# google-research/rigl

Measured on AMD Instinct MI355X. Metric: images/sec/node, ResNet-50 80% ERK RigL step, higher is better.
Workload: dtype bf16

## Files before the change

include/rigl_hip.h:

```cpp
#ifndef RIGL_HIP_H_
#define RIGL_HIP_H_

#include <stddef.h>
#include <stdint.h>

#ifdef __cplusplus
extern "C" {
#endif

#define RIGL_ABI_VERSION 2

typedef void* rigl_stream_t;
typedef uint16_t rigl_bf16;

enum {
  RIGL_OK = 0,
  RIGL_EINVAL = -1,
  RIGL_ELAUNCH = -2,
  RIGL_EWORKSPACE = -3,
  RIGL_EUNSUPPORTED = -4
};

int rigl_version(void);
uint32_t rigl_crc32c(const void* data, size_t n, uint32_t crc);
// ... 383 lines not shown
                           void* workspace, size_t workspace_bytes, rigl_stream_t stream);
int rigl_bn_relu_maxpool_fwd(const RiglConvDesc* d, const rigl_bf16* x,
                             const float* scale, const float* shift, rigl_bf16* y,
                             uint8_t* argmax, rigl_stream_t stream);
size_t rigl_bn_relu_maxpool_bwd_workspace_bytes(const RiglConvDesc* d);
int rigl_bn_relu_maxpool_bwd(const RiglConvDesc* d, const rigl_bf16* x,
                             const rigl_bf16* dy, const uint8_t* argmax,
                             const float* gamma, const float* save_mean,
                             const float* save_invstd, const float* save_scale,
                             const float* save_shift, rigl_bf16* dx, float* dgamma,
                             float* dbeta, void* workspace, size_t workspace_bytes,
                             rigl_stream_t stream);

int rigl_global_avgpool_fwd(int32_t n, int32_t pixels, int32_t c, const rigl_bf16* x,
                            rigl_bf16* y, rigl_stream_t stream);
int rigl_global_avgpool_bwd(int32_t n, int32_t pixels, int32_t c, const rigl_bf16* dy,
                            rigl_bf16* dx, rigl_stream_t stream);
int rigl_global_avgpool_bwd_relu(int32_t n, int32_t pixels, int32_t c, const rigl_bf16* dy,
                                 const rigl_bf16* x, rigl_bf16* dx, rigl_stream_t stream);
int rigl_softmax_xent(int32_t rows, int32_t classes, const rigl_bf16* logits,
                      const int64_t* labels, float label_smoothing, float grad_scale,
                      float* row_loss, rigl_bf16* dlogits , rigl_stream_t stream);

int32_t rigl_conv2d_fwd_takes_relu_epilogue(const RiglConvDesc* d);
int32_t rigl_conv2d_bwd_takes_relu_epilogue(const RiglConvDesc* d);
int rigl_masked_conv2d_fwd_relu(const RiglConvDesc* d, const rigl_bf16* x,
                                const rigl_bf16* w_ohwi, rigl_bf16* y, void* workspace,
                                size_t workspace_bytes, rigl_stream_t stream);
int rigl_masked_conv2d_bwd_relu(const RiglConvDesc* d, const rigl_bf16* x,
                                const rigl_bf16* dy, const rigl_bf16* w_hwio, float* dw,
                                rigl_bf16* dx, void* workspace, size_t workspace_bytes,
                                rigl_stream_t stream);
int rigl_relu_fwd(int64_t n, const rigl_bf16* x, rigl_bf16* y, rigl_stream_t stream);
int rigl_relu_bwd(int64_t n, const rigl_bf16* dy, const rigl_bf16* x, rigl_bf16* dx,
                  rigl_stream_t stream);

typedef struct RiglBnInferItem {
  const float* gamma;
  const float* beta;
  const float* moving_mean;
  const float* moving_variance;
  float* scale_shift;
  int32_t c;
  float eps;
} RiglBnInferItem;
int rigl_bn_infer_params_batched(const RiglBnInferItem* items, int32_t n_items,
// ... 48 lines not shown
```

rigl_amd/_lib.py:

```python
import ctypes as C
import os

_HERE = os.path.dirname(os.path.abspath(__file__))
ABI_VERSION = 2
LIB_PATH = os.environ.get('RIGL_HIP_LIB') or os.path.join(_HERE, 'lib', 'librigl_hip.so')

RIGL_OK = 0
RIGL_EINVAL = -1
RIGL_ELAUNCH = -2
RIGL_EWORKSPACE = -3
RIGL_EUNSUPPORTED = -4
COUNTS_PER_LAYER = 8
MAGPRUNE_COUNTS_PER_LAYER = 4
PROF_KINDS = ('conv_fwd', 'conv_dgrad', 'conv_wgrad', 'prune_regrow',
              'sgd_momentum', 'pack_weights', 'conv_bwd', 'depthwise', 'masked_adam', 'magnitude_prune')

GROW_ZEROS, GROW_GRAD_SCALE, GROW_GRAD_SIGN, GROW_EXPLICIT = 0, 1, 2, 3
MOMRESET_ZEROS, MOMRESET_GRAD = 0, 1


class RiglError(RuntimeError):

  def __init__(self, code, msg):
    super().__init__('librigl_hip: error %d: %s' % (code, msg))
# ... 144 lines not shown
    'rigl_bn_bwd': (C.c_int, [_I64, _I32, _P, _P, _P, _P, _P, _P, _P, _P, _P, _I32, _P, _P, _P, _P, _P, _SZ, _P]),
    'rigl_bn_bwd_stats': (C.c_int, [_I64, _I32, _P, _P, _P, _P, _P, _P, _P, _P, _P, _I32, _P, _P, _P, _P, _P, _I32, _P, _SZ, _P]),
    'rigl_bn_bwd_reduce': (C.c_int, [_I64, _I32, _P, _P, _P, _P, _P, _P, _I32, _P, _P, _P, _P, _SZ, _P]),
    'rigl_crc32c': (C.c_uint32, [_P, _SZ, C.c_uint32]),
    'rigl_stateless_random': (C.c_int, [_P, _I64, _I32, _I32, _I32, _F, _F, _P]),
    'rigl_stateless_random_batched': (C.c_int, [C.POINTER(RandomItem), _I32, _P]),
    'rigl_dropout_fwd': (C.c_int, [_P, _P, _P, _I64, _I32, _F, _I32, _P, _P]),
    'rigl_dropout_bwd': (C.c_int, [_P, _P, _P, _I64, _I32, _F, _P]),
    'rigl_dropout_advance': (C.c_int, [_P, _P]),
    'rigl_cifar_batch': (C.c_int, [_P, _P, _I64, _I32, _I32, _I32, _I32, _I32, _P, _P, _I32, _P, _P, _P]),
    'rigl_cifar_advance': (C.c_int, [_P, _P]),
    'rigl_maxpool_fwd': (C.c_int, [C.POINTER(ConvDesc), _P, _P, _P, _P]),
    'rigl_maxpool_bwd': (C.c_int, [C.POINTER(ConvDesc), _P, _P, _P, _P]),
    'rigl_bn_fwd_statistics': (C.c_int, [_I64, _I32, _P, _P, _P, _P, _P, _F, _F, _P, _P, _P, _P, _P, _I32, _P, _SZ, _P]),
    'rigl_bn_add_bn_fwd': (C.c_int, [_I64, _I32, _P, _P, _P, _P, _P, _P, _P, _P, _F, _F, _I32, _P, _P, _P, _P, _P, _P, _I32, _P, _P, _SZ, _P]),
    'rigl_bn_add_bn_bwd_workspace_bytes': (_SZ, [_I64, _I32]),
    'rigl_bn_add_bn_bwd': (C.c_int, [_I64, _I32, _P, _P, _P, _P, _P, _P, _P, _P, _P, _P, _P, _P, _P, _P, _P, _P, _P, _SZ, _P]),
    'rigl_bn_relu_maxpool_fwd': (C.c_int, [C.POINTER(ConvDesc), _P, _P, _P, _P, _P, _P]),
    'rigl_bn_relu_maxpool_bwd_workspace_bytes': (_SZ, [C.POINTER(ConvDesc)]),
    'rigl_bn_relu_maxpool_bwd': (C.c_int, [C.POINTER(ConvDesc), _P, _P, _P, _P, _P, _P, _P, _P, _P, _P, _P, _P, _SZ, _P]),
    'rigl_global_avgpool_fwd': (C.c_int, [_I32, _I32, _I32, _P, _P, _P]),
    'rigl_global_avgpool_bwd': (C.c_int, [_I32, _I32, _I32, _P, _P, _P]),
    'rigl_softmax_xent': (C.c_int, [_I32, _I32, _P, _P, _F, _F, _P, _P, _P]),
    'rigl_global_avgpool_bwd_relu': (C.c_int, [_I32, _I32, _I32, _P, _P, _P, _P]),
    'rigl_conv2d_fwd_takes_relu_epilogue': (C.c_int32, [C.POINTER(ConvDesc)]),
    'rigl_conv2d_bwd_takes_relu_epilogue': (C.c_int32, [C.POINTER(ConvDesc)]),
    'rigl_masked_conv2d_fwd_relu': (C.c_int, [C.POINTER(ConvDesc), _P, _P, _P, _P, _SZ, _P]),
    'rigl_masked_conv2d_bwd_relu': (C.c_int, [C.POINTER(ConvDesc), _P, _P, _P, _P, _P, _P, _SZ, _P]),
    'rigl_relu_fwd': (C.c_int, [_I64, _P, _P, _P]),
    'rigl_relu_bwd': (C.c_int, [_I64, _P, _P, _P, _P]),
    'rigl_bn_infer_params_batched': (C.c_int, [C.POINTER(BnInferItem), _I32, _P]),
    'rigl_bn_apply': (C.c_int, [_I64, _I32, _P, _P, _P, _I32, _P, _P]),
    'rigl_bn_apply_pair': (C.c_int, [_I64, _I32, _P, _P, _P, _P, _I32, _P, _P]),
    'rigl_bn_relu_maxpool_infer': (C.c_int, [C.POINTER(ConvDesc), _P, _P, _P, _P]),
    'rigl_conv2d_fwd_takes_bn_epilogue': (C.c_int32, [C.POINTER(ConvDesc), _I32, _I32]),
    'rigl_masked_conv2d_fwd_bn_infer': (C.c_int, [C.POINTER(ConvDesc), _P, _P, _P, _P, _P, _I32, _P, _P]),
    'rigl_eval_metrics': (C.c_int, [_I32, _I32, _P, _P, _F, _I32, _P, _P, _P, _P]),
    'rigl_prof_enable': (C.c_int, [_I32]),
    'rigl_prof_collect': (C.c_int, [C.POINTER(C.c_double), C.POINTER(_I64)]),
    'rigl_prof_collect_kinds': (C.c_int, [C.POINTER(C.c_double), C.POINTER(_I64), _I32]),
    'rigl_prof_collect_launches': (C.c_int, [C.POINTER(ProfLaunch), _I64, C.POINTER(_I64)]),
    'rigl_probe_mfma_bf16': (C.c_int, [_I32, _I32, _P, _P]),
    'rigl_tune_set': (C.c_int, [C.c_char_p, _I32]),
    'rigl_tune_get': (_I32, [C.c_char_p, _I32]),
    'rigl_tune_generation': (C.c_uint64, []),
    'rigl_tune_generation_addr': (C.c_void_p, []),
# ... 34 lines not shown
```

rigl_amd/csrc/head.hip:

```cpp
#include "common.hpp"

namespace rigl {
namespace khead {

constexpr int THREADS = 256;

__device__ __forceinline__ float bf_lo(uint32_t v) { return __uint_as_float(v << 16); }
__device__ __forceinline__ float bf_hi(uint32_t v) { return __uint_as_float(v & 0xFFFF0000u); }
__device__ __forceinline__ uint32_t f2bf(float f) {
  uint32_t u = __float_as_uint(f);
  if ((u & 0x7FFFFFFFu) > 0x7F800000u) return (u >> 16) | 0x40u;
  u += 0x7FFFu + ((u >> 16) & 1u);
  return u >> 16;
}
__device__ __forceinline__ float bf16_at(const uint16_t* p, int64_t i) { return __uint_as_float((uint32_t)p[i] << 16); }

__global__ __launch_bounds__(THREADS) void k_avgpool_fwd(int n, int p, int c2, const uint32_t* __restrict__ x,
                                                          uint32_t* __restrict__ y) {
  const int i = blockIdx.x * THREADS + threadIdx.x;
  if (i >= n * c2) return;
  const int img = i / c2, ch = i % c2;
  const uint32_t* src = x + (int64_t)img * p * c2 + ch;
  float a = 0.f, b = 0.f;
  for (int q = 0; q < p; ++q) {
// ... 4 lines not shown
  y[i] = f2bf(a / inv) | (f2bf(b / inv) << 16);
}

__global__ __launch_bounds__(THREADS) void k_avgpool_fwd8(int n, int p, int c8, const uint4* __restrict__ x, uint4* __restrict__ y) {
  const int i = blockIdx.x * THREADS + threadIdx.x;
  if (i >= n * c8) return;
  const int img = i / c8, ch = i % c8;
  const uint4* src = x + (int64_t)img * p * c8 + ch;
  float a[8];
#pragma unroll
  for (int j = 0; j < 8; ++j) a[j] = 0.f;
#pragma unroll 7
  for (int q = 0; q < p; ++q) {
    const uint4 v = src[(int64_t)q * c8];
    a[0] += bf_lo(v.x); a[1] += bf_hi(v.x); a[2] += bf_lo(v.y); a[3] += bf_hi(v.y);
    a[4] += bf_lo(v.z); a[5] += bf_hi(v.z); a[6] += bf_lo(v.w); a[7] += bf_hi(v.w);
  }
  const float inv = (float)p;
  uint4 o;
  o.x = f2bf(a[0] / inv) | (f2bf(a[1] / inv) << 16); o.y = f2bf(a[2] / inv) | (f2bf(a[3] / inv) << 16);
  o.z = f2bf(a[4] / inv) | (f2bf(a[5] / inv) << 16); o.w = f2bf(a[6] / inv) | (f2bf(a[7] / inv) << 16);
  y[i] = o;
}
__global__ __launch_bounds__(THREADS) void k_avgpool_bwd8(int n, int p, int c8, const uint4* __restrict__ dy, uint4* __restrict__ dx) {
  const int64_t total = (int64_t)n * p * c8;
  const float inv = (float)p;
  for (int64_t i = (int64_t)blockIdx.x * THREADS + threadIdx.x; i < total; i += (int64_t)gridDim.x * THREADS) {
    const int ch = (int)(i % c8);
    const int img = (int)(i / ((int64_t)p * c8));
    const uint4 v = dy[(int64_t)img * c8 + ch];
    uint4 o;
    o.x = f2bf(bf_lo(v.x) / inv) | (f2bf(bf_hi(v.x) / inv) << 16); o.y = f2bf(bf_lo(v.y) / inv) | (f2bf(bf_hi(v.y) / inv) << 16);
    o.z = f2bf(bf_lo(v.z) / inv) | (f2bf(bf_hi(v.z) / inv) << 16); o.w = f2bf(bf_lo(v.w) / inv) | (f2bf(bf_hi(v.w) / inv) << 16);
    dx[i] = o;
  }
}

__global__ __launch_bounds__(THREADS) void k_avgpool_bwd8_relu(int n, int p, int c8, const uint4* __restrict__ dy,
                                                               const uint4* __restrict__ x, uint4* __restrict__ dx) {
  const int64_t total = (int64_t)n * p * c8;
  const float inv = (float)p;
  for (int64_t i0 = (int64_t)blockIdx.x * THREADS; i0 < total; i0 += (int64_t)gridDim.x * THREADS) {
    const int64_t i = i0 + threadIdx.x, c = i < total ? i : total - 1;
    const int ch = (int)(c % c8);
    const int img = (int)(c / ((int64_t)p * c8));
    const uint4 v = dy[(int64_t)img * c8 + ch], xv = x[c];
    uint4 o;
    o.x = f2bf(bf_lo(v.x) / inv) | (f2bf(bf_hi(v.x) / inv) << 16); o.y = f2bf(bf_lo(v.y) / inv) | (f2bf(bf_hi(v.y) / inv) << 16);
    o.z = f2bf(bf_lo(v.z) / inv) | (f2bf(bf_hi(v.z) / inv) << 16); o.w = f2bf(bf_lo(v.w) / inv) | (f2bf(bf_hi(v.w) / inv) << 16);
    if (i < total) dx[i] = gate_bf16x8(o, xv);
  }
}

__global__ __launch_bounds__(THREADS) void k_avgpool_bwd(int n, int p, int c2, const uint32_t* __restrict__ dy,
                                                          uint32_t* __restrict__ dx) {
  const int64_t total = (int64_t)n * p * c2;
  for (int64_t i = (int64_t)blockIdx.x * THREADS + threadIdx.x; i < total; i += (int64_t)gridDim.x * THREADS) {
// ... 111 lines not shown
  if ((threadIdx.x & 63) == 0) {
    const int w = threadIdx.x >> 6;
    shv[w] = bv; shi[w] = bi; shc[w] = greater | (nonfinite << 30);
  }
  __syncthreads();
  if (threadIdx.x == 0) {
    int cnt = shc[0] & 0x3FFFFFFF, nf = shc[0] >> 30;
    for (int w = 1; w < THREADS / 64; ++w) {
      if (am_better(shv[w], shi[w], bv, bi)) { bv = shv[w]; bi = shi[w]; }
      cnt += shc[w] & 0x3FFFFFFF; nf |= shc[w] >> 30;
    }
    const bool top1 = inr && bi == (int)lab;
    const bool topkh = inr && isfinite(zlab) && !nf && cnt < topk;
    row_loss[row] = xent_loss(lse, sz, inr ? zlab - m : 0.f, inr, k, 1.f - eps, eps / (float)k);
    row_flags[row] = (top1 ? 1 : 0) | (topkh ? 2 : 0);
    if (counts) {
      atomicAdd(counts, 1ull);
      if (top1) atomicAdd(counts + 1, 1ull);
      if (topkh) atomicAdd(counts + 2, 1ull);
    }
  }
}

}
}

extern "C" {

int rigl_global_avgpool_fwd(int32_t n, int32_t pixels, int32_t c, const rigl_bf16* x, rigl_bf16* y, rigl_stream_t stream) {
  using namespace rigl;
  using namespace rigl::khead;
  if (n <= 0 || pixels <= 0 || c <= 0 || (c & 1)) return fail(RIGL_EINVAL, "rigl_global_avgpool_fwd: need n, pixels > 0 and an even channel count");
  if (!x || !y) return fail(RIGL_EINVAL, "rigl_global_avgpool_fwd: NULL tensor");
  const int c2 = c / 2;
  if ((c & 7) == 0 && ((uintptr_t)x & 15) == 0 && ((uintptr_t)y & 15) == 0) {
    const int c8 = c / 8;
    hipLaunchKernelGGL(k_avgpool_fwd8, dim3((unsigned)((n * c8 + THREADS - 1) / THREADS)), dim3(THREADS), 0, as_stream(stream),
                       n, pixels, c8, reinterpret_cast<const uint4*>(x), reinterpret_cast<uint4*>(y));
    RIGL_CHECK_LAUNCH("rigl_global_avgpool_fwd");
    return RIGL_OK;
  }
  hipLaunchKernelGGL(k_avgpool_fwd, dim3((unsigned)((n * c2 + THREADS - 1) / THREADS)), dim3(THREADS), 0, as_stream(stream),
                     n, pixels, c2, reinterpret_cast<const uint32_t*>(x), reinterpret_cast<uint32_t*>(y));
  RIGL_CHECK_LAUNCH("rigl_global_avgpool_fwd");
  return RIGL_OK;
}

int rigl_global_avgpool_bwd(int32_t n, int32_t pixels, int32_t c, const rigl_bf16* dy, rigl_bf16* dx, rigl_stream_t stream) {
  using namespace rigl;
  using namespace rigl::khead;
  if (n <= 0 || pixels <= 0 || c <= 0 || (c & 1)) return fail(RIGL_EINVAL, "rigl_global_avgpool_bwd: need n, pixels > 0 and an even channel count");
  if (!dy || !dx) return fail(RIGL_EINVAL, "rigl_global_avgpool_bwd: NULL tensor");
  const int c2 = c / 2;
  if ((c & 7) == 0 && ((uintptr_t)dy & 15) == 0 && ((uintptr_t)dx & 15) == 0) {
    const int c8 = c / 8;
    int64_t blocks8 = ((int64_t)n * pixels * c8 + THREADS - 1) / THREADS;
    if (blocks8 > 8192) blocks8 = 8192;
    hipLaunchKernelGGL(k_avgpool_bwd8, dim3((unsigned)blocks8), dim3(THREADS), 0, as_stream(stream), n, pixels, c8,
                       reinterpret_cast<const uint4*>(dy), reinterpret_cast<uint4*>(dx));
    RIGL_CHECK_LAUNCH("rigl_global_avgpool_bwd");
    return RIGL_OK;
  }
  int64_t blocks = ((int64_t)n * pixels * c2 + THREADS - 1) / THREADS;
  if (blocks > 8192) blocks = 8192;
  hipLaunchKernelGGL(k_avgpool_bwd, dim3((unsigned)blocks), dim3(THREADS), 0, as_stream(stream), n, pixels, c2,
                     reinterpret_cast<const uint32_t*>(dy), reinterpret_cast<uint32_t*>(dx));
  RIGL_CHECK_LAUNCH("rigl_global_avgpool_bwd");
  return RIGL_OK;
}

int rigl_global_avgpool_bwd_relu(int32_t n, int32_t pixels, int32_t c, const rigl_bf16* dy, const rigl_bf16* x, rigl_bf16* dx,
                                 rigl_stream_t stream) {
  using namespace rigl;
  using namespace rigl::khead;
  if (n <= 0 || pixels <= 0 || c <= 0 || (c & 7)) return fail(RIGL_EINVAL, "rigl_global_avgpool_bwd_relu: need n, pixels > 0 and c %% 8 == 0");
  if (!dy || !x || !dx) return fail(RIGL_EINVAL, "rigl_global_avgpool_bwd_relu: NULL tensor");
  if (((uintptr_t)dy & 15) || ((uintptr_t)x & 15) || ((uintptr_t)dx & 15))
    return fail(RIGL_EINVAL, "rigl_global_avgpool_bwd_relu: tensors must be 16-byte aligned");
  const int c8 = c / 8;
  int64_t blocks = ((int64_t)n * pixels * c8 + THREADS - 1) / THREADS;
  if (blocks > 8192) blocks = 8192;
  hipLaunchKernelGGL(k_avgpool_bwd8_relu, dim3((unsigned)blocks), dim3(THREADS), 0, as_stream(stream), n, pixels, c8,
                     reinterpret_cast<const uint4*>(dy), reinterpret_cast<const uint4*>(x), reinterpret_cast<uint4*>(dx));
  RIGL_CHECK_LAUNCH("rigl_global_avgpool_bwd_relu");
  return RIGL_OK;
}

int rigl_softmax_xent(int32_t rows, int32_t classes, const rigl_bf16* logits, const int64_t* labels, float label_smoothing,
                      float grad_scale, float* row_loss, rigl_bf16* dlogits, rigl_stream_t stream) {
  using namespace rigl;
  using namespace rigl::khead;
  if (rows <= 0 || classes <= 0) return fail(RIGL_EINVAL, "rigl_softmax_xent: rows and classes must be positive");
  if (!logits || !labels || !row_loss) return fail(RIGL_EINVAL, "rigl_softmax_xent: NULL tensor");
  if (!(label_smoothing >= 0.f) || label_smoothing > 1.f) return fail(RIGL_EINVAL, "rigl_softmax_xent: label_smoothing %g not in [0,1]", (double)label_smoothing);
  hipLaunchKernelGGL(k_softmax_xent, dim3((unsigned)rows), dim3(THREADS), 0, as_stream(stream), classes, logits, labels,
                     label_smoothing, grad_scale, row_loss, dlogits);
  RIGL_CHECK_LAUNCH("rigl_softmax_xent");
  return RIGL_OK;
}

int rigl_eval_metrics(int32_t rows, int32_t classes, const rigl_bf16* logits, const int64_t* labels, float label_smoothing,
                      int32_t topk, float* row_loss, int32_t* row_flags, int64_t* counts, rigl_stream_t stream) {
  using namespace rigl;
  using namespace rigl::khead;
  if (rows <= 0 || classes <= 0) return fail(RIGL_EINVAL, "rigl_eval_metrics: rows and classes must be positive");
  if (!logits || !labels || !row_loss || !row_flags) return fail(RIGL_EINVAL, "rigl_eval_metrics: NULL tensor");
  if (!(label_smoothing >= 0.f) || label_smoothing > 1.f) return fail(RIGL_EINVAL, "rigl_eval_metrics: label_smoothing %g not in [0,1]", (double)label_smoothing);
  if (topk < 1) return fail(RIGL_EINVAL, "rigl_eval_metrics: topk %d < 1", topk);
  if (classes > EVAL_MAX_CLASSES) return fail(RIGL_EUNSUPPORTED, "rigl_eval_metrics: %d classes > %d (the row is staged in LDS)", classes, EVAL_MAX_CLASSES);
  hipLaunchKernelGGL(k_eval_metrics, dim3((unsigned)rows), dim3(THREADS), (size_t)classes * 4, as_stream(stream), classes, logits,
                     labels, label_smoothing, topk, row_loss, row_flags, reinterpret_cast<unsigned long long*>(counts));
  RIGL_CHECK_LAUNCH("rigl_eval_metrics");
  return RIGL_OK;
}

}
```

rigl_amd/ops.py:

```python
import ctypes as C
import os

import torch

from rigl_amd import _lib
from rigl_amd._lib import (ConvDesc, PackLayer, PruneRegrowLayer,
                           PruneRegrowParams, RiglError, check)

_workspaces = {}


_raw_stream = getattr(torch._C, '_cuda_getCurrentRawStream', None)
_cur_device = getattr(torch._C, '_cuda_getDevice', None)


def _stream():
  if _raw_stream is not None and _cur_device is not None:
    return C.c_void_p(_raw_stream(_cur_device()))
  return C.c_void_p(torch.cuda.current_stream().cuda_stream)


def _ptr(t):
  return C.c_void_p(t.data_ptr()) if t is not None else C.c_void_p(0)

# ... 1023 lines not shown
  _req(x, torch.bfloat16, 'x')
  n, h, w, c = x.shape
  if tuple(dy.shape) != (n, c):
    raise ValueError('dy must be [N, C] of x')
  dx = torch.empty_like(x)
  check(_lib.load().rigl_global_avgpool_bwd_relu(n, h * w, c, _ptr(dy), _ptr(x), _ptr(dx), _stream()))
  return dx


def softmax_xent(logits, labels, label_smoothing=0.0, grad_scale=None, want_grad=True):
  _req(logits, torch.bfloat16, 'logits')
  _req(labels, torch.int64, 'labels')
  rows, k = logits.shape
  if labels.numel() != rows:
    raise ValueError('softmax_xent: %d labels for %d rows' % (labels.numel(), rows))
  loss = torch.empty(rows, dtype=torch.float32, device=logits.device)
  dz = torch.empty_like(logits) if want_grad else None
  check(_lib.load().rigl_softmax_xent(rows, k, _ptr(logits), _ptr(labels), float(label_smoothing),
                                      1.0 / rows if grad_scale is None else float(grad_scale), _ptr(loss), _ptr(dz),
                                      _stream()))
  return loss, dz


def bn_infer_params(bns, out=None):
  bns = list(bns)
  if not bns:
    return []
  total = sum(2 * b.moving_mean.numel() for b in bns)
  dev = bns[0].moving_mean.device
  if out is None:
    out = torch.empty(total, dtype=torch.float32, device=dev)
  _req(out, torch.float32, 'out')
  if out.numel() < total:
    raise ValueError('bn_infer_params: out holds %d floats < %d' % (out.numel(), total))
  arr = (_lib.BnInferItem * len(bns))()
  views, off = [], 0
  for i, b in enumerate(bns):
    c = b.moving_mean.numel()
    for t, nm in ((b.gamma.data, 'gamma'), (b.beta.data, 'beta'), (b.moving_mean, 'moving_mean'),
                  (b.moving_variance, 'moving_variance')):
      _req(t, torch.float32, nm)
      if t.numel() != c:
        raise ValueError('bn_infer_params: %s has %d channels, not %d' % (nm, t.numel(), c))
    v = out[off:off + 2 * c].view(2, c)
    arr[i] = _lib.BnInferItem(b.gamma.data.data_ptr(), b.beta.data.data_ptr(), b.moving_mean.data_ptr(),
                              b.moving_variance.data_ptr(), v.data_ptr(), c, float(b.eps))
# ... 111 lines not shown
```

rigl_amd/pruning_layers.py:

```python
import math
import os

import numpy as np
import torch

from rigl_amd import ops
from rigl_amd import variables as V


def _same_pad(size, k, stride):
  out = -(-size // stride)
  total = max((out - 1) * stride + k - size, 0)
  return out, total // 2


def _valid_out(size, k, stride):
  return (size - k) // stride + 1


_BN_FUSE_BWD = os.environ.get('RIGL_BN_FUSE_BWD', '0') == '1'
_CONV_PAIR = os.environ.get('RIGL_CONV_PAIR', '1') != '0'
_BN_FUSE_MAX_BYTES = float(os.environ.get('RIGL_BN_FUSE_MAX_MB', '1e9')) * 1e6


def _bn_source(x):
  h = getattr(x, 'bn_ctx', None) if _BN_FUSE_BWD else None
  if h is not None:
    h.attached += 1
  return h


def _bn_fuse_request(holder, need_dx):
  if holder is None or not need_dx or holder.attached != 1 or holder.x is None:
    return None
  if holder.x.numel() * 2 > _BN_FUSE_MAX_BYTES:
    return None
  return dict(x=holder.x, saved=holder.saved, relu=holder.relu, relu_bits=holder.bits)


def _bn_fuse_publish(holder, req, dx):
  if req is not None and req.get('partials') is not None and dx is not None:
    holder.partials, holder.dx_ptr = req['partials'], dx.data_ptr()


class _HandOver:
  __slots__ = ('armed', 'grad', 'payload')
  knob = did = None

  def __init__(self):
    self.armed = False
    self.grad = self.payload = None

  def fill(self, grad, *payload):
    self.grad, self.payload = grad, payload

  def take(self, grad):
    filled, payload = self.grad, self.payload
    self.grad = self.payload = None
    if self.armed != (filled is not None):
      raise RuntimeError('%s: the batch norm %s but the forward had decided otherwise' % (self.knob, self.did[filled is None]))
    if filled is None:
      return None
    if grad is not filled and (grad is None or grad.data_ptr() != filled.data_ptr() or grad.shape != filled.shape
                               or not grad.is_contiguous()):
      raise RuntimeError('%s: the gradient that reached the conv is not the one the batch norm handed over' % self.knob)
    return payload


class BnApplyHolder(_HandOver):
  __slots__ = ()
  knob, did = 'bn_bwd_on_load', ('skipped its apply pass', 'ran its apply pass')


class MaskedAddendHolder(_HandOver):
  __slots__ = ()
  knob, did = 'lazy_res_grad', ('handed the shortcut gradient over unmasked', 'wrote the masked shortcut gradient')


def _conv_forward(lv, desc, x, want_stats):
  if x.dtype == torch.float32:
    return ops.conv_fwd_f32(desc, x, lv.weights.data.view(-1), _mask_bits(lv)), None
  return ops.conv_fwd(desc, x, lv.ohwi, stats=True) if want_stats else (ops.conv_fwd(desc, x, lv.ohwi), None)


def stats_outputs(ctx, want_stats, outs, parts, device):
  if not want_stats:
    return outs if len(outs) > 1 else outs[0]
  parts = tuple(p if p is not None else torch.empty(0, device=device) for p in parts)
  ctx.mark_non_differentiable(*parts)
  ctx.set_materialize_grads(False)
  return outs + parts


def _dw_ready(lv):
  sync = getattr(lv.weights.graph, 'grad_sync', None)
  return (lambda: sync.notify_layer_grad_ready(lv.weights)) if sync is not None else None


def _dy_or_zeros(dy, d, x):
  if dy is None:
    return torch.zeros((d.n, d.ho, d.wo, d.cout), dtype=x.dtype, device=x.device)
  return dy.contiguous()


def _mask_bits(lv):
  return lv.mask.bits if lv.mask is not None else None


class _MaskedConvFn(torch.autograd.Function):

  @staticmethod
  def forward(ctx, x, lv, desc, need_dx, want_stats=False, bn_holder=None, pending=None, apply_holder=None):
    ctx.lv, ctx.desc, ctx.need_dx = lv, desc, need_dx
    ctx.bn_holder, ctx.apply_holder = bn_holder, apply_holder
    ctx.save_for_backward(x)
    if pending is not None:
      out = ops.conv_fwd_bnrelu(desc, pending.x, pending.saved, lv.ohwi, x, stats=want_stats)
      y, part = out if want_stats else (out, None)
    else:
      y, part = _conv_forward(lv, desc, x, want_stats)
    return stats_outputs(ctx, want_stats, (y,), (part,), x.device)

  @staticmethod
  def backward(ctx, dy, _dpart=None):
    (x,) = ctx.saved_tensors
    lv, d = ctx.lv, ctx.desc
    dy = _dy_or_zeros(dy, d, x)
    ready = _dw_ready(lv)
    if x.dtype == torch.float32:
      dx = ops.conv_bwd_f32(d, x, dy, lv.weights.data.view(-1), _mask_bits(lv), lv.weights.grad.view(-1),
                            need_dx=ctx.need_dx, on_dw_ready=ready)
      return (dx,) + (None,) * 7
    got = ctx.apply_holder.take(dy) if ctx.apply_holder is not None else None
    if got is not None:
      dx = ops.conv_bwd_bnapply(d, x, dy, lv.hwio, lv.weights.grad.view(-1), *got, on_dw_ready=ready)
      return (dx,) + (None,) * 7
    req = _bn_fuse_request(ctx.bn_holder, ctx.need_dx)
    dx = ops.conv_bwd(d, x, dy, lv.hwio, lv.weights.grad.view(-1), need_dx=ctx.need_dx, on_dw_ready=ready, bn_fuse=req)
    _bn_fuse_publish(ctx.bn_holder, req, dx)
    return (dx,) + (None,) * 7


class _MaskedConvReluFn(torch.autograd.Function):

  @staticmethod
  def forward(ctx, x, lv, desc, need_dx, gate_input):
    ctx.lv, ctx.desc, ctx.need_dx, ctx.gate_input = lv, desc, need_dx, gate_input
    ctx.save_for_backward(x)
    return ops.conv_fwd_relu(desc, x, lv.ohwi)

  @staticmethod
  def backward(ctx, dy):
    (x,) = ctx.saved_tensors
    lv, d = ctx.lv, ctx.desc
    dy, ready = _dy_or_zeros(dy, d, x), _dw_ready(lv)
    if ctx.need_dx and ctx.gate_input:
      dx = ops.conv_bwd_relu(d, x, dy, lv.hwio, lv.weights.grad.view(-1), on_dw_ready=ready)
    else:
      dx = ops.conv_bwd(d, x, dy, lv.hwio, lv.weights.grad.view(-1), need_dx=ctx.need_dx, on_dw_ready=ready)
    return dx, None, None, None, None


class _MaskedConvForkFn(torch.autograd.Function):
# ... 205 lines not shown

  def __init__(self, graph, scope, n_in, units, use_bias=True,
               sparsity_technique='baseline', weight_decay=0.0,
               kernel_initializer=None, activation=None):
    super().__init__(graph, scope, (n_in, units), sparsity_technique,
                     weight_decay, kernel_initializer)
    self.n_in, self.units = n_in, units
    self.activation = activation
    self._descs = {}
    if use_bias:
      self.bias = graph.add_variable(scope + '/biases', (units,), V.KIND_OTHER, 0.0)

  def __call__(self, x):
    if x.shape[-1] != self.n_in:
      raise ValueError('expected %d inputs, got %d' % (self.n_in, x.shape[-1]))
    self.graph.refresh_shadows()
    lead = x.shape[:-1]
    x2 = x.reshape(-1, 1, 1, self.n_in)
    b = x2.shape[0]
    d = self._descs.get(b)
    if d is None:
      d = ops.conv_desc(b, 1, 1, self.n_in, self.units, 1, 1, 1, 0, 0, 1, 1)
      self._descs[b] = d
    need_dx = x2.requires_grad
    if not x2.requires_grad:
      x2 = x2.detach().requires_grad_(True)
    y = _MaskedConvFn.apply(x2.contiguous(), self.vars, d, need_dx)
    y = y.reshape(*lead, self.units)
    if self.bias is not None:
      y = y + bias_tensor(self.bias).to(y.dtype)
    if self.activation is not None:
      y = self.activation(y)
    return y


def bias_tensor(var):
  leaf = getattr(var, '_leaf', None)
  if leaf is None or leaf.data_ptr() != var.data.data_ptr():
    leaf = var.data.detach().requires_grad_(True)
    var._leaf = leaf
  if leaf.grad is None or leaf.grad.data_ptr() != var.grad.data_ptr():
    leaf.grad = var.grad
  return leaf


_init_rng = np.random.RandomState(0)


def set_init_seed(seed):
  global _init_rng
  _init_rng = np.random.RandomState(seed)


def variance_scaling_initializer(scale=1.0):

# ... 89 lines not shown
```

rigl_amd/workloads/nn.py:

```python
import os

import torch
import torch.nn.functional as F

from rigl_amd import variables as V
from rigl_amd.pruning_layers import bias_tensor, stats_outputs

BATCH_NORM_DECAY = 0.9
BATCH_NORM_EPSILON = 1e-5
_DW_STATS = os.environ.get('RIGL_DW_STATS', '1') != '0'


def activation_dtype(precision=None):
  if precision is None:
    from rigl_amd import ops
    precision = 'float32' if ops.tune_get('k1_fp32', 0) == 1 else 'bfloat16'
  if precision not in ('bfloat16', 'float32'):
    raise ValueError('precision must be bfloat16 or float32, got %r' % (precision,))
  return torch.float32 if precision == 'float32' else torch.bfloat16


def nchw_view(x):
  return x.permute(0, 3, 1, 2)

# ... 418 lines not shown

  @staticmethod
  def forward(ctx, x):
    from rigl_amd import ops
    ctx.save_for_backward(x)
    return ops.global_avgpool_fwd(x)

  @staticmethod
  def backward(ctx, dy):
    from rigl_amd import ops
    (x,) = ctx.saved_tensors
    return ops.global_avgpool_bwd_relu(dy.contiguous(), x)


def global_avg_pool_relu(x):
  if not (x.is_cuda and x.dtype == torch.bfloat16 and x.dim() == 4 and x.shape[-1] % 8 == 0):
    raise ValueError('global_avg_pool_relu: a bf16 [N, H, W, C] GPU tensor with C % 8 == 0')
  return _GlobalAvgPoolReluFn.apply(x.contiguous())


class _SoftmaxXentFn(torch.autograd.Function):

  @staticmethod
  def forward(ctx, logits, labels, label_smoothing):
    from rigl_amd import ops
    rows, dz = ops.softmax_xent(logits.contiguous(), labels.reshape(-1).contiguous(), label_smoothing)
    ctx.save_for_backward(dz)
    return rows.mean()

  @staticmethod
  def backward(ctx, g):
    dz, = ctx.saved_tensors
    return (dz * g.to(dz.dtype)), None, None


def softmax_cross_entropy(logits, labels, label_smoothing=0.0):
  if (_HEAD_KERNELS and logits.is_cuda and logits.dtype == torch.bfloat16 and logits.dim() == 2 and
      labels.dtype == torch.int64):
    return _SoftmaxXentFn.apply(logits, labels, float(label_smoothing))
  logp = F.log_softmax(logits.float(), dim=-1)
  nll = -logp.gather(1, labels.reshape(-1, 1)).squeeze(1)
  if not label_smoothing:
    return nll.mean()
  k = logits.shape[-1]
  return ((1.0 - label_smoothing) * nll - (label_smoothing / k) * logp.sum(dim=1)).mean()
```

Baseline: 12810.

## Add fused classifier head FC kernels and fold loss scale into backward

Adds dedicated MFMA-based forward and backward kernels for the final dense classifier layer. The forward fuses the bias add. The backward computes dW, dbias and dx in a single launch and applies the loss-gradient scale inside the kernel, so the separate elementwise dz*g multiply and generic conv paths are skipped via a new loss-scale handover. The avgpool backward is also restructured to broadcast per image over pixel groups using nontemporal stores. This adds new code paths and checks, but the head is a tiny part of a ResNet-50 step.

```diff
diff --git a/include/rigl_hip.h b/include/rigl_hip.h
--- a/include/rigl_hip.h
+++ b/include/rigl_hip.h
@@ -429,6 +429,13 @@
                       const int64_t* labels, float label_smoothing, float grad_scale,
                       float* row_loss, rigl_bf16* dlogits , rigl_stream_t stream);
 
+int rigl_head_fc_fwd(int32_t n, int32_t k, int32_t c, const rigl_bf16* x, const rigl_bf16* w_ohwi,
+                     const float* bias , rigl_bf16* logits, rigl_stream_t stream);
+int rigl_head_fc_bwd(int32_t n, int32_t k, int32_t c, const rigl_bf16* x, const rigl_bf16* dz,
+                     const float* gscale , const rigl_bf16* w_hwio,
+                     rigl_bf16* dx , float* dw, float* dbias ,
+                     rigl_stream_t stream);
+
 int32_t rigl_conv2d_fwd_takes_relu_epilogue(const RiglConvDesc* d);
 int32_t rigl_conv2d_bwd_takes_relu_epilogue(const RiglConvDesc* d);
 int rigl_masked_conv2d_fwd_relu(const RiglConvDesc* d, const rigl_bf16* x,
diff --git a/rigl_amd/_lib.py b/rigl_amd/_lib.py
--- a/rigl_amd/_lib.py
+++ b/rigl_amd/_lib.py
@@ -190,6 +190,8 @@
     'rigl_global_avgpool_fwd': (C.c_int, [_I32, _I32, _I32, _P, _P, _P]),
     'rigl_global_avgpool_bwd': (C.c_int, [_I32, _I32, _I32, _P, _P, _P]),
     'rigl_softmax_xent': (C.c_int, [_I32, _I32, _P, _P, _F, _F, _P, _P, _P]),
+    'rigl_head_fc_fwd': (C.c_int, [_I32, _I32, _I32, _P, _P, _P, _P, _P]),
+    'rigl_head_fc_bwd': (C.c_int, [_I32, _I32, _I32, _P, _P, _P, _P, _P, _P, _P, _P]),
     'rigl_global_avgpool_bwd_relu': (C.c_int, [_I32, _I32, _I32, _P, _P, _P, _P]),
     'rigl_conv2d_fwd_takes_relu_epilogue': (C.c_int32, [C.POINTER(ConvDesc)]),
     'rigl_conv2d_bwd_takes_relu_epilogue': (C.c_int32, [C.POINTER(ConvDesc)]),
diff --git a/rigl_amd/csrc/head.hip b/rigl_amd/csrc/head.hip
--- a/rigl_amd/csrc/head.hip
+++ b/rigl_amd/csrc/head.hip
@@ -50,17 +50,19 @@
   o.z = f2bf(a[4] / inv) | (f2bf(a[5] / inv) << 16); o.w = f2bf(a[6] / inv) | (f2bf(a[7] / inv) << 16);
   y[i] = o;
 }
-__global__ __launch_bounds__(THREADS) void k_avgpool_bwd8(int n, int p, int c8, const uint4* __restrict__ dy, uint4* __restrict__ dx) {
-  const int64_t total = (int64_t)n * p * c8;
+typedef __attribute__((ext_vector_type(4))) unsigned int u32x4;
+__global__ __launch_bounds__(THREADS) void k_avgpool_bwd8(int n, int p, int c8, int per, int pgroups, const uint4* __restrict__ dy,
+                                                           u32x4* __restrict__ dx) {
+  const int img = blockIdx.x / pgroups, q0 = (blockIdx.x % pgroups) * per;
+  const int q1 = q0 + per < p ? q0 + per : p;
   const float inv = (float)p;
-  for (int64_t i = (int64_t)blockIdx.x * THREADS + threadIdx.x; i < total; i += (int64_t)gridDim.x * THREADS) {
-    const int ch = (int)(i % c8);
-    const int img = (int)(i / ((int64_t)p * c8));
+  for (int ch = threadIdx.x; ch < c8; ch += THREADS) {
     const uint4 v = dy[(int64_t)img * c8 + ch];
-    uint4 o;
+    u32x4 o;
     o.x = f2bf(bf_lo(v.x) / inv) | (f2bf(bf_hi(v.x) / inv) << 16); o.y = f2bf(bf_lo(v.y) / inv) | (f2bf(bf_hi(v.y) / inv) << 16);
     o.z = f2bf(bf_lo(v.z) / inv) | (f2bf(bf_hi(v.z) / inv) << 16); o.w = f2bf(bf_lo(v.w) / inv) | (f2bf(bf_hi(v.w) / inv) << 16);
-    dx[i] = o;
+    u32x4* dst = dx + ((int64_t)img * p + q0) * c8 + ch;
+    for (int q = q0; q < q1; ++q, dst += c8) __builtin_nontemporal_store(o, dst);
   }
 }
 
@@ -218,6 +220,182 @@
   }
 }
 
+typedef __attribute__((ext_vector_type(8))) __bf16 bf16x8;
+typedef __attribute__((ext_vector_type(4))) float f32x4;
+typedef short s16x4 __attribute__((ext_vector_type(4)));
+typedef short s16x8 __attribute__((ext_vector_type(8)));
+
+constexpr int FC_ROWS = 64;
+constexpr int FC_FWD_WAVES = 8;
+constexpr int FC_DW_ROWB = 144;
+constexpr int FC_SMEM = 2 * 64 * FC_DW_ROWB;
+
+__device__ __forceinline__ uint32_t scale_bf16x2(uint32_t v, float gs) { return f2bf(bf_lo(v) * gs) | (f2bf(bf_hi(v) * gs) << 16); }
+__device__ __forceinline__ uint4 scale_bf16x8(uint4 v, float gs) {
+  return make_uint4(scale_bf16x2(v.x, gs), scale_bf16x2(v.y, gs), scale_bf16x2(v.z, gs), scale_bf16x2(v.w, gs));
+}
+
+template <bool SCALE, int NW, int U>
+__device__ __forceinline__ void fc_nt_tile(int M, int J, int R, const uint16_t* __restrict__ P, const uint16_t* __restrict__ Q, int m0,
+                                           int j0, float gs, const float* __restrict__ bias, uint16_t* __restrict__ out, float* red) {
+  const int lane = threadIdx.x & 63, wave = threadIdx.x >> 6, g = lane >> 4, li = lane & 15;
+  const int nsteps = (R + 31) >> 5, r8 = R >> 3;
+  const int rem = nsteps % (2 * NW) - 2 * wave;
+  const int ns = 2 * (nsteps / (2 * NW)) + (rem < 0 ? 0 : rem > 2 ? 2 : rem);
+  const int jq = j0 + li < J ? j0 + li : J - 1;
+  const uint16_t* qrow = Q + (int64_t)jq * R;
+  const uint16_t* prow[4];
+#pragma unroll
+  for (int t = 0; t < 4; ++t) {
+    const int m = m0 + 16 * t + li;
+    prow[t] = P + (int64_t)(m < M ? m : M - 1) * R;
+  }
+  f32x4 acc[4];
+#pragma unroll
+  for (int t = 0; t < 4; ++t) acc[t] = f32x4{0.f, 0.f, 0.f, 0.f};
+  const uint4 zero = make_uint4(0u, 0u, 0u, 0u);
+  for (int i0 = 0; i0 < ns; i0 += U) {
+    uint4 fq[U], fp[U][4];
+#pragma unroll
+    for (int u = 0; u < U; ++u) {
+      const int i = i0 + u < ns ? i0 + u : ns - 1;
+      const int ch = 4 * (2 * NW * (i >> 1) + 2 * wave + (i & 1)) + g;
+      const bool ok = ch < r8;
+      const int off = ok ? ch * 8 : 0;
+      fq[u] = *reinterpret_cast<const uint4*>(qrow + off);
+#pragma unroll
+      for (int t = 0; t < 4; ++t) fp[u][t] = *reinterpret_cast<const uint4*>(prow[t] + off);
+      if (!ok) {
+        fq[u] = zero;
+#pragma unroll
+        for (int t = 0; t < 4; ++t) fp[u][t] = zero;
+      }
+    }
+#pragma unroll
+    for (int u = 0; u < U; ++u) {
+      if (i0 + u < ns) {
+        const bf16x8 a = __builtin_bit_cast(bf16x8, fq[u]);
+#pragma unroll
+        for (int t = 0; t < 4; ++t) {
+          const uint4 pv = SCALE ? scale_bf16x8(fp[u][t], gs) : fp[u][t];
+          acc[t] = __builtin_amdgcn_mfma_f32_16x16x32_bf16(a, __builtin_bit_cast(bf16x8, pv), acc[t], 0, 0, 0);
+        }
+      }
+    }
+  }
+  f32x4* red4 = reinterpret_cast<f32x4*>(red);
+#pragma unroll
+  for (int t = 0; t < 4; ++t) red4[(wave * 4 + t) * 64 + lane] = acc[t];
+  __syncthreads();
+  if (wave >= 4) return;
+  f32x4 s = red4[wave * 64 + lane];
+#pragma unroll
+  for (int v = 1; v < NW; ++v) s += red4[(v * 4 + wave) * 64 + lane];
+  const int m = m0 + 16 * wave + li, j = j0 + 4 * g;
+  if (m < M && j < J) {
+    uint32_t o[4];
+#pragma unroll
+    for (int r = 0; r < 4; ++r) {
+      o[r] = f2bf(s[r]);
+      if (bias) o[r] = f2bf(__uint_as_float(o[r] << 16) + __uint_as_float(f2bf(bias[j + r]) << 16));
+    }
+    *reinterpret_cast<uint2*>(out + (int64_t)m * J + j) = make_uint2(o[0] | (o[1] << 16), o[2] | (o[3] << 16));
+  }
+}
+
+__device__ __forceinline__ bf16x8 fc_read_tr_pair(const unsigned char* p0, const unsigned char* p1) {
+  const s16x4 lo = __builtin_amdgcn_ds_read_tr16_b64_v4i16((s16x4 __attribute__((address_space(3)))*)p0);
+  const s16x4 hi = __builtin_amdgcn_ds_read_tr16_b64_v4i16((s16x4 __attribute__((address_space(3)))*)p1);
+  return __builtin_bit_cast(bf16x8, __builtin_shufflevector(lo, hi, 0, 1, 2, 3, 4, 5, 6, 7));
+}
+
+template <bool SCALE>
+__device__ __forceinline__ void fc_dw_tile(int n, int k, int c, const uint16_t* __restrict__ x, const uint16_t* __restrict__ dz, float gs,
+                                           float* __restrict__ dw, float* __restrict__ dbias, int k0, int c0, unsigned char* smem) {
+  unsigned char* Xs = smem;
+  unsigned char* Ds = smem + 64 * FC_DW_ROWB;
+  const int tid = threadIdx.x, lane = tid & 63, wave = tid >> 6, g = lane >> 4, li = lane & 15;
+  const int srow = tid >> 3, sch = tid & 7;
+  const bool dok = c0 + 8 * sch < c;
+  const uint4 zero = make_uint4(0u, 0u, 0u, 0u);
+  uint4 rx[2], rd[2];
+  auto fetch = [&](int nb) {
+#pragma unroll
+    for (int i = 0; i < 2; ++i) {
+      const int r = nb * 64 + srow + 32 * i;
+      rx[i] = r < n ? *reinterpret_cast<const uint4*>(x + (int64_t)r * k + k0 + 8 * sch) : zero;
+      rd[i] = (r < n && dok) ? *reinterpret_cast<const uint4*>(dz + (int64_t)r * c + c0 + 8 * sch) : zero;
+      if (SCALE) rd[i] = scale_bf16x8(rd[i], gs);
+    }
+  };
+  fetch(0);
+  f32x4 acc[4];
+#pragma unroll
+  for (int t = 0; t < 4; ++t) acc[t] = f32x4{0.f, 0.f, 0.f, 0.f};
+  float bsum = 0.f;
+  const bool do_bias = dbias != nullptr && k0 == 0 && tid < 64;
+  const int tr_off = (8 * g + (li >> 2)) * FC_DW_ROWB + 8 * (li & 3);
+  const int nchunks = (n + 63) >> 6;
+  for (int nb = 0; nb < nchunks; ++nb) {
+    if (nb) __syncthreads();
+#pragma unroll
+    for (int i = 0; i < 2; ++i) {
+      *reinterpret_cast<uint4*>(Xs + (srow + 32 * i) * FC_DW_ROWB + 16 * sch) = rx[i];
+      *reinterpret_cast<uint4*>(Ds + (srow + 32 * i) * FC_DW_ROWB + 16 * sch) = rd[i];
+    }
+    __syncthreads();
+    if (nb + 1 < nchunks) fetch(nb + 1);
+#pragma unroll
+    for (int s = 0; s < 2; ++s) {
+      const int base = s * 32 * FC_DW_ROWB + tr_off;
+      const bf16x8 xb = fc_read_tr_pair(Xs + base + 32 * wave, Xs + base + 4 * FC_DW_ROWB + 32 * wave);
+#pragma unroll
+      for (int t = 0; t < 4; ++t) {
+        const bf16x8 da = fc_read_tr_pair(Ds + base + 32 * t, Ds + base + 4 * FC_DW_ROWB + 32 * t);
+        acc[t] = __builtin_amdgcn_mfma_f32_16x16x32_bf16(da, xb, acc[t], 0, 0, 0);
+      }
+    }
+    if (do_bias) {
+      const int rows = n - nb * 64 < 64 ? n - nb * 64 : 64;
+      for (int r = 0; r < rows; ++r) bsum += bf16_at(reinterpret_cast<const uint16_t*>(Ds + r * FC_DW_ROWB), tid);
+    }
+  }
+  const int kk = k0 + 16 * wave + li;
+#pragma unroll
+  for (int t = 0; t < 4; ++t) {
+    const int cc = c0 + 16 * t + 4 * g;
+    if (cc < c) *reinterpret_cast<f32x4*>(dw + (int64_t)kk * c + cc) = acc[t];
+  }
+  if (do_bias && c0 + tid < c) dbias[c0 + tid] += __uint_as_float(f2bf(bsum) << 16);
+}
+
+__global__ __launch_bounds__(FC_FWD_WAVES * 64) void k_head_fc_fwd(int n, int k, int c, const uint16_t* __restrict__ x,
+                                                          const uint16_t* __restrict__ w_ohwi, const float* __restrict__ bias,
+                                                          uint16_t* __restrict__ logits) {
+  __shared__ __align__(16) float red[FC_FWD_WAVES * 4 * 64 * 4];
+  fc_nt_tile<false, FC_FWD_WAVES, 8>(n, c, k, x, w_ohwi, blockIdx.y * FC_ROWS, blockIdx.x * 16, 1.f, bias, logits, red);
+}
+
+__global__ __launch_bounds__(THREADS) void k_head_fc_bwd(int n, int k, int c, const uint16_t* __restrict__ x,
+                                                          const uint16_t* __restrict__ dz, const float* __restrict__ gscale,
+                                                          const uint16_t* __restrict__ w_hwio, uint16_t* __restrict__ dx,
+                                                          float* __restrict__ dw, float* __restrict__ dbias, int n_dw) {
+  __shared__ __align__(16) unsigned char smem[FC_SMEM];
+  const float gs = gscale ? __uint_as_float(f2bf(*gscale) << 16) : 1.f;
+  const int b = blockIdx.x;
+  if (b < n_dw) {
+    const int nct = (c + 63) >> 6;
+    const int k0 = (b / nct) * 64, c0 = (b % nct) * 64;
+    if (gscale) fc_dw_tile<true>(n, k, c, x, dz, gs, dw, dbias, k0, c0, smem);
+    else fc_dw_tile<false>(n, k, c, x, dz, gs, dw, dbias, k0, c0, smem);
+  } else {
+    const int kt = k >> 4;
+    const int j0 = ((b - n_dw) % kt) * 16, m0 = ((b - n_dw) / kt) * FC_ROWS;
+    if (gscale) fc_nt_tile<true, 4, 4>(n, k, c, dz, w_hwio, m0, j0, gs, nullptr, dx, reinterpret_cast<float*>(smem));
+    else fc_nt_tile<false, 4, 4>(n, k, c, dz, w_hwio, m0, j0, gs, nullptr, dx, reinterpret_cast<float*>(smem));
+  }
+}
+
 }
 }
 
@@ -250,10 +428,12 @@
   const int c2 = c / 2;
   if ((c & 7) == 0 && ((uintptr_t)dy & 15) == 0 && ((uintptr_t)dx & 15) == 0) {
     const int c8 = c / 8;
-    int64_t blocks8 = ((int64_t)n * pixels * c8 + THREADS - 1) / THREADS;
-    if (blocks8 > 8192) blocks8 = 8192;
-    hipLaunchKernelGGL(k_avgpool_bwd8, dim3((unsigned)blocks8), dim3(THREADS), 0, as_stream(stream), n, pixels, c8,
-                       reinterpret_cast<const uint4*>(dy), reinterpret_cast<uint4*>(dx));
+    int pgroups = (2048 + n - 1) / n;
+    if (pgroups > pixels) pgroups = pixels;
+    const int per = (pixels + pgroups - 1) / pgroups;
+    pgroups = (pixels + per - 1) / per;
+    hipLaunchKernelGGL(k_avgpool_bwd8, dim3((unsigned)((int64_t)n * pgroups)), dim3(THREADS), 0, as_stream(stream), n, pixels, c8, per,
+                       pgroups, reinterpret_cast<const uint4*>(dy), reinterpret_cast<u32x4*>(dx));
     RIGL_CHECK_LAUNCH("rigl_global_avgpool_bwd");
     return RIGL_OK;
   }
@@ -295,6 +475,54 @@
   return RIGL_OK;
 }
 
+static int head_fc_check(const char* who, int32_t n, int32_t k, int32_t c) {
+  using namespace rigl;
+  if (n < 1 || n > 256 || k < 64 || (k % 64) || c < 8 || (c % 8))
+    return fail(RIGL_EINVAL, "%s: n %d, k %d, c %d: need 1 <= n <= 256, k %% 64 == 0 and c %% 8 == 0", who, n, k, c);
+  return RIGL_OK;
+}
+static bool head_fc_aligned(const void* p) { return ((uintptr_t)p & 15) == 0; }
+
+int rigl_head_fc_fwd(int32_t n, int32_t k, int32_t c, const rigl_bf16* x, const rigl_bf16* w_ohwi, const float* bias, rigl_bf16* logits,
+                     rigl_stream_t stream) {
+  using namespace rigl;
+  using namespace rigl::khead;
+  const char* who = "rigl_head_fc_fwd";
+  if (int rc = head_fc_check(who, n, k, c)) return rc;
+  if (!x || !w_ohwi || !logits) return fail(RIGL_EINVAL, "%s: NULL tensor", who);
+  if (!head_fc_aligned(x) || !head_fc_aligned(w_ohwi) || !head_fc_aligned(logits))
+    return fail(RIGL_EINVAL, "%s: tensors must be 16-byte aligned", who);
+  const RiglConvDesc d = {n, 1, 1, k, 1, 1, c, 1, 1, 1, 1, 0, 0};
+  prof_set_tag(&d);
+  ProfFamily prof(PROF_CONV_FWD);
+  RIGL_K_LAUNCH(k_head_fc_fwd, dim3((unsigned)((c + 15) / 16), (unsigned)((n + FC_ROWS - 1) / FC_ROWS)), dim3(FC_FWD_WAVES * 64),
+                0, as_stream(stream), n, k, c, reinterpret_cast<const uint16_t*>(x), reinterpret_cast<const uint16_t*>(w_ohwi), bias,
+                reinterpret_cast<uint16_t*>(logits));
+  RIGL_CHECK_LAUNCH(who);
+  return RIGL_OK;
+}
+
+int rigl_head_fc_bwd(int32_t n, int32_t k, int32_t c, const rigl_bf16* x, const rigl_bf16* dz, const float* gscale,
+                     const rigl_bf16* w_hwio, rigl_bf16* dx, float* dw, float* dbias, rigl_stream_t stream) {
+  using namespace rigl;
+  using namespace rigl::khead;
+  const char* who = "rigl_head_fc_bwd";
+  if (int rc = head_fc_check(who, n, k, c)) return rc;
+  if (!x || !dz || !dw || (dx && !w_hwio)) return fail(RIGL_EINVAL, "%s: NULL tensor", who);
+  if (!head_fc_aligned(x) || !head_fc_aligned(dz) || !head_fc_aligned(w_hwio) || !head_fc_aligned(dx) || !head_fc_aligned(dw))
+    return fail(RIGL_EINVAL, "%s: tensors must be 16-byte aligned", who);
+  const RiglConvDesc d = {n, 1, 1, k, 1, 1, c, 1, 1, 1, 1, 0, 0};
+  prof_set_tag(&d);
+  ProfFamily prof(PROF_CONV_BWD);
+  const int n_dw = (k / 64) * ((c + 63) / 64);
+  const int n_dx = dx ? (k / 16) * ((n + FC_ROWS - 1) / FC_ROWS) : 0;
+  RIGL_K_LAUNCH(k_head_fc_bwd, dim3((unsigned)(n_dw + n_dx)), dim3(THREADS), 0, as_stream(stream), n, k, c,
+                reinterpret_cast<const uint16_t*>(x), reinterpret_cast<const uint16_t*>(dz), gscale,
+                reinterpret_cast<const uint16_t*>(w_hwio), reinterpret_cast<uint16_t*>(dx), dw, dbias, n_dw);
+  RIGL_CHECK_LAUNCH(who);
+  return RIGL_OK;
+}
+
 int rigl_eval_metrics(int32_t rows, int32_t classes, const rigl_bf16* logits, const int64_t* labels, float label_smoothing,
                       int32_t topk, float* row_loss, int32_t* row_flags, int64_t* counts, rigl_stream_t stream) {
   using namespace rigl;
diff --git a/rigl_amd/ops.py b/rigl_amd/ops.py
--- a/rigl_amd/ops.py
+++ b/rigl_amd/ops.py
@@ -1069,6 +1069,58 @@
   return loss, dz
 
 
+def head_fc_legal(n, k, c):
+  return 1 <= n <= 256 and k >= 64 and k % 64 == 0 and c >= 8 and c % 8 == 0
+
+
+def head_fc_on():
+  return tune_get('head_fc', 1) != 0
+
+
+def _aligned16(*ts):
+  return all(t is None or t.data_ptr() % 16 == 0 for t in ts)
+
+
+def head_fc_fwd(d, x, w_ohwi, bias=None, logits=None):
+  _req(x, torch.bfloat16, 'x')
+  _req(w_ohwi, torch.bfloat16, 'w_ohwi')
+  _req(bias, torch.float32, 'bias', allow_none=True)
+  n, k, c = d.n, d.cin, d.cout
+  if x.numel() != n * k or w_ohwi.numel() != k * c or (bias is not None and bias.numel() != c):
+    raise ValueError('head_fc_fwd: x must be [%d, %d], w_ohwi [%d, %d] and bias [%d]' % (n, k, c, k, c))
+  _count_macs('fwd_macs', d)
+  logits = _out(logits, (n, c), torch.bfloat16, x.device, 'logits')
+  check(_lib.load().rigl_head_fc_fwd(n, k, c, _ptr(x), _ptr(w_ohwi), _ptr(bias), _ptr(logits), _stream()))
+  return logits
+
+
+def head_fc_bwd(d, x, dz, w_hwio, dw, dbias=None, gscale=None, need_dx=True, on_dw_ready=None, dx=None):
+  _req(x, torch.bfloat16, 'x')
+  _req(dz, torch.bfloat16, 'dz')
+  _req(dw, torch.float32, 'dw')
+  _req(dbias, torch.float32, 'dbias', allow_none=True)
+  _req(gscale, torch.float32, 'gscale', allow_none=True)
+  n, k, c = d.n, d.cin, d.cout
+  if x.numel() != n * k or dz.numel() != n * c or dw.numel() != k * c or (dbias is not None and dbias.numel() != c):
+    raise ValueError('head_fc_bwd: x must be [%d, %d], dz [%d, %d], dw [%d, %d] and dbias [%d]' % (n, k, n, c, k, c, c))
+  if gscale is not None and gscale.numel() != 1:
+    raise ValueError('head_fc_bwd: gscale must hold one float')
+  _count_macs('wgrad_macs', d)
+  if need_dx:
+    _req(w_hwio, torch.bfloat16, 'w_hwio')
+    if w_hwio.numel() != k * c:
+      raise ValueError('head_fc_bwd: w_hwio must be [%d, %d]' % (k, c))
+    _count_macs('dgrad_macs', d)
+    dx = _out(dx, (n, k), torch.bfloat16, dz.device, 'dx')
+  else:
+    dx = None
+  check(_lib.load().rigl_head_fc_bwd(n, k, c, _ptr(x), _ptr(dz), _ptr(gscale), _ptr(w_hwio) if need_dx else _ptr(None),
+                                     _ptr(dx), _ptr(dw), _ptr(dbias), _stream()))
+  if on_dw_ready is not None:
+    on_dw_ready()
+  return dx
+
+
 def bn_infer_params(bns, out=None):
   bns = list(bns)
   if not bns:
diff --git a/rigl_amd/pruning_layers.py b/rigl_amd/pruning_layers.py
--- a/rigl_amd/pruning_layers.py
+++ b/rigl_amd/pruning_layers.py
@@ -46,6 +46,7 @@
 class _HandOver:
   __slots__ = ('armed', 'grad', 'payload')
   knob = did = None
+  giver, taker = 'the batch norm', 'the conv'
 
   def __init__(self):
     self.armed = False
@@ -53,17 +54,21 @@
 
   def fill(self, grad, *payload):
     self.grad, self.payload = grad, payload
+
+  @staticmethod
+  def _same(grad, filled):
+    return grad is filled or (grad is not None and grad.data_ptr() == filled.data_ptr() and grad.shape == filled.shape
+                              and grad.is_contiguous())
 
   def take(self, grad):
     filled, payload = self.grad, self.payload
     self.grad = self.payload = None
     if self.armed != (filled is not None):
-      raise RuntimeError('%s: the batch norm %s but the forward had decided otherwise' % (self.knob, self.did[filled is None]))
+      raise RuntimeError('%s: %s %s but the forward had decided otherwise' % (self.knob, self.giver, self.did[filled is None]))
     if filled is None:
       return None
-    if grad is not filled and (grad is None or grad.data_ptr() != filled.data_ptr() or grad.shape != filled.shape
-                               or not grad.is_contiguous()):
-      raise RuntimeError('%s: the gradient that reached the conv is not the one the batch norm handed over' % self.knob)
+    if not self._same(grad, filled):
+      raise RuntimeError('%s: the gradient that reached %s is not the one %s handed over' % (self.knob, self.taker, self.giver))
     return payload
 
 
@@ -75,6 +80,16 @@
 class MaskedAddendHolder(_HandOver):
   __slots__ = ()
   knob, did = 'lazy_res_grad', ('handed the shortcut gradient over unmasked', 'wrote the masked shortcut gradient')
+
+
+class LossScaleHolder(_HandOver):
+  __slots__ = ()
+  knob, did = 'head_fc', ('handed its gradient over', 'did not hand its gradient over')
+  giver, taker = 'the loss', 'the classifier'
+
+  @staticmethod
+  def _same(grad, filled):
+    return grad is not None and grad.data_ptr() == filled.data_ptr() and grad.numel() == filled.numel() and grad.is_contiguous()
 
 
 def _conv_forward(lv, desc, x, want_stats):
@@ -114,6 +129,9 @@
     ctx.lv, ctx.desc, ctx.need_dx = lv, desc, need_dx
     ctx.bn_holder, ctx.apply_holder = bn_holder, apply_holder
     ctx.save_for_backward(x)
+    head = getattr(ctx, 'head', None)
+    if head is not None:
+      return ops.head_fc_fwd(desc, x, lv.ohwi, head[0].data if head[0] is not None else None).view(desc.n, 1, 1, desc.cout)
     if pending is not None:
       out = ops.conv_fwd_bnrelu(desc, pending.x, pending.saved, lv.ohwi, x, stats=want_stats)
       y, part = out if want_stats else (out, None)
@@ -131,6 +149,13 @@
       dx = ops.conv_bwd_f32(d, x, dy, lv.weights.data.view(-1), _mask_bits(lv), lv.weights.grad.view(-1),
                             need_dx=ctx.need_dx, on_dw_ready=ready)
       return (dx,) + (None,) * 7
+    head = getattr(ctx, 'head', None)
+    if head is not None:
+      bias, holder = head
+      got = holder.take(dy)
+      dx = ops.head_fc_bwd(d, x, dy, lv.hwio, lv.weights.grad.view(-1), bias.grad if bias is not None else None,
+                           gscale=got[0] if got is not None else None, need_dx=ctx.need_dx, on_dw_ready=ready)
+      return (dx.view(x.shape) if dx is not None else None,) + (None,) * 7
     got = ctx.apply_holder.take(dy) if ctx.apply_holder is not None else None
     if got is not None:
       dx = ops.conv_bwd_bnapply(d, x, dy, lv.hwio, lv.weights.grad.view(-1), *got, on_dw_ready=ready)
@@ -139,6 +164,18 @@
     dx = ops.conv_bwd(d, x, dy, lv.hwio, lv.weights.grad.view(-1), need_dx=ctx.need_dx, on_dw_ready=ready, bn_fuse=req)
     _bn_fuse_publish(ctx.bn_holder, req, dx)
     return (dx,) + (None,) * 7
+
+
+class _HeadDenseFn(torch.autograd.Function):
+
+  @staticmethod
+  def forward(ctx, x, lv, desc, need_dx, bias, holder):
+    ctx.head = (bias, holder)
+    return _MaskedConvFn.forward(ctx, x, lv, desc, need_dx)
+
+  @staticmethod
+  def backward(ctx, dz):
+    return _MaskedConvFn.backward(ctx, dz)[:1] + (None,) * 5
 
 
 class _MaskedConvReluFn(torch.autograd.Function):
@@ -390,6 +427,8 @@
     if d is None:
       d = ops.conv_desc(b, 1, 1, self.n_in, self.units, 1, 1, 1, 0, 0, 1, 1)
       self._descs[b] = d
+    if self._takes_head_fc(x, b):
+      return self._head_fc(x, d)
     need_dx = x2.requires_grad
     if not x2.requires_grad:
       x2 = x2.detach().requires_grad_(True)
@@ -399,6 +438,26 @@
       y = y + bias_tensor(self.bias).to(y.dtype)
     if self.activation is not None:
       y = self.activation(y)
+    return y
+
+  def _takes_head_fc(self, x, b):
+    if not (x.dim() == 2 and x.is_cuda and x.dtype == torch.bfloat16 and ops.head_fc_legal(b, self.n_in, self.units)):
+      return False
+    lv, bias = self.vars, self.bias
+    if bias is not None and not (bias.data.dtype == torch.float32 and bias.grad is not None and bias.grad.is_contiguous()):
+      return False
+    return ops.head_fc_on() and ops._aligned16(x, lv.ohwi, lv.hwio, lv.weights.grad)
+
+  def _head_fc(self, x, d):
+    need_dx = x.requires_grad
+    if not need_dx:
+      x = x.detach().requires_grad_(True)
+    holder = LossScaleHolder()
+    y = _HeadDenseFn.apply(x.reshape(-1, 1, 1, self.n_in).contiguous(), self.vars, d, need_dx, self.bias, holder)
+    y = y.reshape(-1, self.units)
+    if self.activation is not None:
+      return self.activation(y)
+    y.loss_scale = holder
     return y
 
 
diff --git a/rigl_amd/workloads/nn.py b/rigl_amd/workloads/nn.py
--- a/rigl_amd/workloads/nn.py
+++ b/rigl_amd/workloads/nn.py
@@ -464,22 +464,33 @@
 class _SoftmaxXentFn(torch.autograd.Function):
 
   @staticmethod
-  def forward(ctx, logits, labels, label_smoothing):
+  def forward(ctx, logits, labels, label_smoothing, scale_holder=None):
     from rigl_amd import ops
     rows, dz = ops.softmax_xent(logits.contiguous(), labels.reshape(-1).contiguous(), label_smoothing)
     ctx.save_for_backward(dz)
+    ctx.scale_holder = scale_holder
+    if scale_holder is not None:
+      scale_holder.armed = True
     return rows.mean()
 
   @staticmethod
   def backward(ctx, g):
     dz, = ctx.saved_tensors
-    return (dz * g.to(dz.dtype)), None, None
+    h = ctx.scale_holder
+    if h is None:
+      return (dz * g.to(dz.dtype)), None, None, None
+    if g.is_cuda and g.dtype == torch.float32 and g.numel() == 1 and g.is_contiguous():
+      h.fill(dz, g)
+      return dz, None, None, None
+    dzs = dz * g.to(dz.dtype)
+    h.fill(dzs, None)
+    return dzs, None, None, None
 
 
 def softmax_cross_entropy(logits, labels, label_smoothing=0.0):
   if (_HEAD_KERNELS and logits.is_cuda and logits.dtype == torch.bfloat16 and logits.dim() == 2 and
       labels.dtype == torch.int64):
-    return _SoftmaxXentFn.apply(logits, labels, float(label_smoothing))
+    return _SoftmaxXentFn.apply(logits, labels, float(label_smoothing), getattr(logits, 'loss_scale', None))
   logp = F.log_softmax(logits.float(), dim=-1)
   nll = -logp.gather(1, labels.reshape(-1, 1)).squeeze(1)
   if not label_smoothing:
```

Result: no change. 12860, median of 6 (+0.4%).
